# ChaoyueSong/MoDA

Measured on AMD Instinct MI355X. Metric: rays/s (256 samples/ray, 8x256 MLP, 25 bones), higher is better.
Workload: dtype f16

## Files before the change

### moda_amd/csrc/mlp_fused.hip

```cpp
#include <hip/hip_runtime.h>
#include <stdint.h>

#include <atomic>
#include <type_traits>

#include "moda_hip.h"
#include "moda_dev.h"

namespace {

typedef float f32x16 __attribute__((ext_vector_type(16)));
typedef float f32x4 __attribute__((ext_vector_type(4)));
typedef __bf16 bf16x8 __attribute__((ext_vector_type(8)));
typedef _Float16 f16x8 __attribute__((ext_vector_type(8)));

#ifndef MODA_BF16_WAVES
#define MODA_BF16_WAVES 8
#endif
#ifndef MODA_BF16_CB128
#define MODA_BF16_CB128 2
#endif
#ifndef MODA_BF16_CB
#define MODA_BF16_CB 1
#endif
#ifndef MODA_BF16_CB64
#define MODA_BF16_CB64 1
#endif
#ifndef MODA_BF16_WAVES64
#define MODA_BF16_WAVES64 16
#endif
#ifndef MODA_RING
#define MODA_RING 6
#endif
#ifndef MODA_STAGGER
#define MODA_STAGGER 0
#endif
#ifndef MODA_RESIDENT
#define MODA_RESIDENT 1
#endif
#ifndef MODA_APIPE
#define MODA_APIPE 2
#endif
#ifndef MODA_HEAD_PREFETCH
#define MODA_HEAD_PREFETCH 0
#endif
#ifndef MODA_DMA_LEADERS
#define MODA_DMA_LEADERS 0
#endif
#ifndef MODA_DMA_SPLIT
#define MODA_DMA_SPLIT 0
#endif
#ifndef MODA_XLAYER
#define MODA_XLAYER 0
#endif
#ifndef MODA_X3_EPI_PIPE
#define MODA_X3_EPI_PIPE 0
#endif
#ifndef MODA_X3_WAVES256
#define MODA_X3_WAVES256 4
#endif
#ifndef MODA_X3_WAVES128
#define MODA_X3_WAVES128 4
#endif
#ifndef MODA_X3_WAVES
#define MODA_X3_WAVES 8
#endif
#ifndef MODA_RING_SAFE
#define MODA_RING_SAFE 1
#endif
#ifndef MODA_F16_TRACK
#define MODA_F16_TRACK 1
#endif
#ifndef MODA_AGPR_APIPE
#define MODA_AGPR_APIPE 4
#endif
#ifndef MODA_AGPR_PREFETCH
#define MODA_AGPR_PREFETCH 0
// ... 704 lines not shown
        return (qi & 2) ? -r : r;
    }
    static DEVINL void encode(Pe& p, float x, float y, float z, int h, const float* win_lds) {
        float v[32];
#pragma unroll
        for (int q = 0; q < 30; ++q) {
            const int k = q / 3;
            const int c = q - 3 * k;
            const float t = (c == 0 ? x : (c == 1 ? y : z)) * (float)(1 << k);
            v[q] = win_lds[k] * sin_quarter_shifted(t, h);
        }
        v[30] = h ? y : x;
        v[31] = h ? 0.f : z;
#pragma unroll
        for (int g = 0; g < PEG; ++g) {
            union { u32x4_ w; bf16x8 b; } oh, ol;
#pragma unroll
            for (int q = 0; q < 4; ++q) {
                unsigned hi, lo;
                split_pk(v[8 * g + 2 * q], v[8 * g + 2 * q + 1], hi, lo);
                oh.w[q] = hi;
                ol.w[q] = lo;
            }
            p.hi[g] = oh.b;
            p.lo[g] = ol.b;
        }
    }
};

DEVINL float sigmoidf(float v) { return 1.f / (1.f + expf(-v)); }
DEVINL void keep_alive(const f32x16& v) { asm volatile("" ::"v"(v)); }

template <int W, typename P, int CB, int NWAVES, bool ENDY, bool UNI, bool WARP = false, int DUMP = 0, int RING = MODA_RING,
          bool COMP = false, bool HX = false>
__global__ __launch_bounds__(NWAVES * 64) __attribute__((amdgpu_waves_per_eu(NWAVES / 4, NWAVES / 4)))
void mlp_fused_kernel(MlpArgs a) {
    static_assert(!HX || (kIsF16<P> && ((WARP && W == 64) || (!WARP && W == 256 && DUMP == 0 && !COMP))),
                  "split heads: the fp16 skin + warp kernel and the fp16 8 x 256 kernel");
    constexpr bool HXR = HX && !WARP;
    static_assert(!COMP || (UNI && !WARP && DUMP == 0 && CB == 1 && std::is_same<P, PrecBF16>::value),
                  "the compositing epilogue is built for the bf16 UNI inference kernels");
    static_assert(!WARP || (UNI && !std::is_same<P, PrecF32>::value), "the warp epilogue is built for the bf16-geometry UNI kernels");
    static_assert(!DUMP || (std::is_same<P, PrecBF16>::value && !WARP), "activation dumps are built for the bf16 kernels");
    constexpr int NTHREADS = NWAVES * 64;
    constexpr int NT = W / 32;
    constexpr int NTD = (NT / 2 > 0) ? NT / 2 : 1;
    constexpr int CHF = (W == 64) ? 8 : 16;
    constexpr int TILE = NWAVES * 32 * CB;
    constexpr bool RESIDENT = (W == 64) && kIs16<P> && (MODA_RESIDENT != 0);
    using RingT = Ring<CHF, NWAVES, RESIDENT, RING, kAsmMfma<P>>;
    const int ring_chunks = RESIDENT ? a.nchunks : RING;

    extern __shared__ __attribute__((aligned(16))) unsigned char smem[];
    float* bias_lds = (float*)(smem + ring_chunks * RingT::kChunkBytes);
    float* win_lds = bias_lds + a.nbias;
    constexpr int RBW = 2 * W + NTD * 32;
    float* rb_slots = win_lds + 16;
    f32x4* pe_lds = (f32x4*)(rb_slots + NWAVES * CB * RBW) + threadIdx.x;
    constexpr int PE_VEC = sizeof(typename P::Pe) / 16;
    constexpr int TBW = (DUMP == 4) ? 2048 : 4096;
    constexpr int TBRS = (DUMP == 4) ? 64 : 128;
    unsigned char* const tbuf = (unsigned char*)(rb_slots + NWAVES * CB * RBW) + sizeof(typename P::Pe) * CB * NTHREADS +
                                (threadIdx.x >> 6) * (CB * TBW);

    const int lane = threadIdx.x & 63;
    const int wave = __builtin_amdgcn_readfirstlane(threadIdx.x >> 6);
    const int col = lane & 31;
    const int h = lane >> 5;

    for (int i = threadIdx.x; i < a.nbias; i += NTHREADS) bias_lds[i] = a.bias[i];
    if (threadIdx.x < 16) win_lds[threadIdx.x] = a.window[threadIdx.x];
    __syncthreads();

    RingT ring;
    ring.rsrc = __builtin_amdgcn_make_buffer_rsrc((void*)a.wstream, 0, a.nchunks * RingT::kChunkBytes, 0x00020000);
    ring.lds = smem;
    ring.nchunks = a.nchunks;
    ring.lane = lane;
    ring.wave = wave;
    ring.leader = wave < NWAVES / 2;
    ring.prime();
    constexpr int PREQ = (kAsmMfma<P> && MODA_AGPR_PREQ != 0) ? MODA_AGPR_APIPE : 0;
    typename P::Frag preq[PREQ > 0 ? PREQ : 1];
    auto prefetch_next = [&]() __attribute__((always_inline)) {
        if constexpr (PREQ > 0) {
#pragma unroll
            for (int d = 0; d < PREQ; ++d) preq[d] = P::fetch(ring);
        }
    };
    prefetch_next();

    const bool with_sigma = (a.flags & (MODA_MLP_WITH_SIGMA | MODA_MLP_SIGMA_ONLY)) != 0;
    const bool sigma_only = (a.flags & MODA_MLP_SIGMA_ONLY) != 0;
    const bool do_sigmoid = (a.flags & MODA_MLP_SIGMOID) != 0;
    const int nout_t = (a.n_out + 31) >> 5;
    const int n_mid = a.n_pre + 1 + a.n_post;

#ifdef MODA_STAMPS
    unsigned long long stamp_acc[16] = {0};
    unsigned long long stamp_prev;
    asm volatile("s_memtime %0\n\ts_waitcnt lgkmcnt(0)" : "=s"(stamp_prev)::"memory");
#endif
    const int ntiles = (a.M + TILE - 1) / TILE;
    unsigned trk = 0u;
    struct Head {
        float x, y, z;
        f32x4 rb[3];
    };
    auto sample_at = [&](int t, int cb, bool& ok) __attribute__((always_inline)) {
        const int mm = t * TILE + wave * (32 * CB) + cb * 32 + col;
        ok = mm < a.M;
        return ok ? mm : a.M - 1;
    };
    auto row_at = [&](int t, int cb, int div, int R) __attribute__((always_inline)) {
        bool ok;
        const unsigned r = (unsigned)sample_at(t, cb, ok) / (unsigned)div;
        return (int)(r < (unsigned)R ? r : (unsigned)R - 1u);
    };
    auto load_head = [&](int t, int cb, bool uni) __attribute__((always_inline)) {
        Head hd;
        hd.rb[0] = hd.rb[1] = hd.rb[2] = f32x4{0.f, 0.f, 0.f, 0.f};
        int r1u = __builtin_amdgcn_readfirstlane(row_at(t, cb, a.div1, a.R1));
        const int rdu = __builtin_amdgcn_readfirstlane(row_at(t, cb, a.divd, a.Rd));
        if constexpr (WARP) {
            if (a.rows_at_runs) r1u = a.run_start[r1u];
        }
#ifndef MODA_ABL_NOHEADLOAD
        if (uni) {
            if (lane < W / 4) {
                hd.rb[0] = *(const f32x4*)(a.rb1 + (long long)r1u * W + 4 * lane);
                hd.rb[1] = *(const f32x4*)(a.rb5 + (long long)r1u * W + 4 * lane);
            }
            if (lane < NTD * 8 && (a.flags & MODA_MLP_SIGMA_ONLY) == 0)
                hd.rb[2] = *(const f32x4*)(a.rbd + (long long)rdu * (NTD * 32) + 4 * lane);
        }
#endif
        bool ok;
        const long long mm = sample_at(t, cb, ok);
#ifdef MODA_ABL_NOHEADLOAD
        hd.x = 0.001f * (float)(mm & 1023);
        hd.y = 0.002f * (float)(lane);
        hd.z = 0.3f;
#else
        hd.x = a.xyz[mm * 3 + 0];
        hd.y = a.xyz[mm * 3 + 1];
        hd.z = a.xyz[mm * 3 + 2];
#endif
        if (a.flip != nullptr && a.flip[mm]) hd.x = -hd.x;
        return hd;
    };
    constexpr bool PREFETCH = UNI && ((MODA_HEAD_PREFETCH != 0) || (kAsmMfma<P> && MODA_AGPR_PREFETCH != 0)) && (DUMP == 0);
    Head head[CB];
    if (PREFETCH) {
#pragma unroll
        for (int cb = 0; cb < CB; ++cb) head[cb] = load_head(blockIdx.x, cb, true);
    }
    for (int tile = blockIdx.x; tile < ntiles; tile += gridDim.x) {
        STAMP(15);
        if (UNI && a.n_live != nullptr) {
            bool any_live = false;
#pragma unroll
            for (int cb = 0; cb < CB; ++cb) {
                const int m_first = tile * TILE + wave * (32 * CB) + cb * 32;
                if (m_first < a.M) {
                    const int ray = m_first / a.live_S;
                    any_live = any_live || (m_first - ray * a.live_S) < a.n_live[ray];
                }
            }
            if (!__builtin_amdgcn_readfirstlane((int)any_live)) {
                for (int c = 0; c < a.nchunks; ++c) {
                    ring.acquire();
                    ring.issue_rest();
                    ring.advance();
                }
                if (PREFETCH) {
#pragma unroll
                    for (int cb = 0; cb < CB; ++cb) head[cb] = load_head(tile + gridDim.x, cb, true);
                }
                continue;
            }
        }
        auto sample_of = [&](int cb, bool& ok) __attribute__((always_inline)) { return sample_at(tile, cb, ok); };
        auto row_of = [&](int cb, int div, int R) __attribute__((always_inline)) { return row_at(tile, cb, div, R); };
        bool rb_uni[CB];
#pragma unroll
        for (int cb = 0; cb < CB; ++cb) {
            if (UNI) {
                rb_uni[cb] = true;
            } else {
                const int r1 = row_of(cb, a.div1, a.R1), rd = row_of(cb, a.divd, a.Rd);
                const int r1u = __builtin_amdgcn_readfirstlane(r1), rdu = __builtin_amdgcn_readfirstlane(rd);
                rb_uni[cb] = __builtin_amdgcn_ballot_w64(r1 != r1u || rd != rdu) == 0ull;
            }
            if (!PREFETCH) head[cb] = load_head(tile, cb, rb_uni[cb]);
        }
        typename P::Pe pe[CB];
#pragma unroll
        for (int cb = 0; cb < CB; ++cb) P::encode(pe[cb], head[cb].x, head[cb].y, head[cb].z, h, win_lds);
#pragma unroll
        for (int cb = 0; cb < CB; ++cb) {
            float* slot = rb_slots + (wave * CB + cb) * RBW;
            if (rb_uni[cb]) {
                if (lane < W / 4) {
                    *(f32x4*)(slot + 4 * lane) = head[cb].rb[0];
                    *(f32x4*)(slot + W + 4 * lane) = head[cb].rb[1];
                }
                if (lane < NTD * 8) *(f32x4*)(slot + 2 * W + 4 * lane) = head[cb].rb[2];
            }
        }
        if (PREFETCH) {
#pragma unroll
            for (int cb = 0; cb < CB; ++cb) head[cb] = load_head(tile + gridDim.x, cb, true);
        }
        float comp_z = 0.f, comp_delta = 0.f, comp_noise_v = 0.f, comp_ib = 0.f;
        if constexpr (COMP) {
            bool okc;
            const int mmc = sample_of(0, okc);
            const int nc = mmc / a.comp_S, sxc = mmc - nc * a.comp_S;
            comp_z = a.comp_zv[mmc];
            comp_delta = (sxc + 1 < a.comp_S ? a.comp_zv[mmc + 1] - comp_z : 1e10f) * comp_dnorm(a.comp_rd, nc);
            comp_noise_v = a.comp_noise ? a.comp_noise[mmc] : 0.f;
            comp_ib = comp_ibeta(a.comp_beta);
        }
        STAMP(0);

        typename P::Act actX[CB][NT], actY[CB][NT];
#pragma unroll
        for (int cb = 0; cb < CB; ++cb)
#pragma unroll
            for (int t = 0; t < NT; ++t) {
                P::fresh_act(actX[cb][t]);
                P::fresh_act(actY[cb][t]);
                if constexpr (kAsmMfma<P>) {
                    actX[cb][t].base = P::kRegX + cb * P::kRegBlock + t * P::kRegTile;
                    actY[cb][t].base = P::kRegY + cb * P::kRegBlock + t * P::kRegTile;
                }
            }

        auto init_glob = [&](f32x16& c, const float* rb, int row, int ld, int rt) __attribute__((always_inline)) {
            const float* p = rb + (long long)row * ld + 32 * rt + 4 * h;
#pragma unroll
            for (int q = 0; q < 4; ++q) {
                const f32x4 v = *(const f32x4*)(p + 8 * q);
#pragma unroll
                for (int i = 0; i < 4; ++i) c[4 * q + i] = v[i];
// ... 297 lines not shown
            if constexpr (PREQ > 0) {
                ring.end_layer();
                prefetch_next();
            }
#pragma unroll
            for (int cb = 0; cb < CB; ++cb) settle_acc<P>(accs[cb]);
        }
        if constexpr (PREQ == 0) ring.end_layer();
#pragma unroll
        for (int cb = 0; cb < CB; ++cb) P::note(trk, accs[cb][0]);
        if (sigma_only) {
#pragma unroll
            for (int cb = 0; cb < CB; ++cb) {
                bool ok;
                const long long mm = sample_of(cb, ok);
                if (ok && h == 0) a.out[mm * a.out_stride] = accs[cb][0];
            }
            continue;
        }
        boff += (NT + 1) * 32;
        STAMP(7);

        typename P::Act actd[CB][NTD];
        if constexpr (kAsmMfma<P>) {
            static_assert(!kAsmMfma<P> || (CB == 2 && NT == 8 && NWAVES == 4 && !WARP && DUMP == 0 && !COMP), "the AGPR map of PrecBF16A / PrecF16A");
#pragma unroll
            for (int cb = 0; cb < CB; ++cb)
#pragma unroll
                for (int t = 0; t < NTD; ++t) {
                    actd[cb][t].base = (ENDY ? P::kRegX : P::kRegY) + cb * P::kRegBlock + t * P::kRegTile;
                    if constexpr (HXR) actd_lo[cb][t].base = actd[cb][t].base + NTD * P::kRegTile;
                }
        }
        f32x16 acco[CB][2];
        if constexpr (HX && WARP) {
            f32x16 accd[CB];
#pragma unroll
            for (int cb = 0; cb < CB; ++cb) init_rowbias(accd[cb], cb, 2, 0);
#pragma unroll
            for (int t = 0; t < NT; ++t)
#pragma unroll
                for (int sb = 0; sb < P::SUBS; ++sb) {
                    const f32x4 whi = ring.next(), wlo = ring.next();
#pragma unroll
                    for (int cb = 0; cb < CB; ++cb) {
                        accd[cb] = __builtin_amdgcn_mfma_f32_32x32x16_f16(P::as_f16(wlo), hid[cb][t].b[sb], accd[cb], 0, 0, 0);
                        accd[cb] = __builtin_amdgcn_mfma_f32_32x32x16_f16(P::as_f16(whi), hid[cb][t].b[sb], accd[cb], 0, 0, 0);
                    }
                }
            ring.end_layer();
            typename P::Act actd_lo[CB];
#pragma unroll
            for (int cb = 0; cb < CB; ++cb) {
                P::note(trk, accd[cb][0]);
#pragma unroll
                for (int u = 0; u < 2; ++u) {
                    union { typename P::u32x4 w; f16x8 b; } oh, ol;
#pragma unroll
                    for (int q = 0; q < 4; ++q) {
                        const float v0 = fmaxf(accd[cb][8 * u + 2 * q], 0.f), v1 = fmaxf(accd[cb][8 * u + 2 * q + 1], 0.f);
                        const unsigned hi = P::cvt_pk(v0, v1);
                        union { unsigned u; _Float16 h[2]; } hh;
                        hh.u = hi;
                        oh.w[q] = hi;
                        ol.w[q] = P::cvt_pk(v0 - (float)hh.h[0], v1 - (float)hh.h[1]);
                    }
                    actd[cb][0].b[u] = oh.b;
                    actd_lo[cb].b[u] = ol.b;
                }
            }
#pragma unroll
            for (int ot = 0; ot < 2; ++ot)
#pragma unroll
                for (int cb = 0; cb < CB; ++cb) init_lds(acco[cb][ot], bias_lds + boff, ot);
#pragma unroll
            for (int ot = 0; ot < 2; ++ot) {
                if (ot < nout_t) {
#pragma unroll
                    for (int sb = 0; sb < P::SUBS; ++sb) {
                        const f32x4 whi = ring.next(), wlo = ring.next();
#pragma unroll
                        for (int cb = 0; cb < CB; ++cb) {
                            acco[cb][ot] = __builtin_amdgcn_mfma_f32_32x32x16_f16(P::as_f16(wlo), actd[cb][0].b[sb], acco[cb][ot], 0, 0, 0);
                            acco[cb][ot] = __builtin_amdgcn_mfma_f32_32x32x16_f16(P::as_f16(whi), actd_lo[cb].b[sb], acco[cb][ot], 0, 0, 0);
                            acco[cb][ot] = __builtin_amdgcn_mfma_f32_32x32x16_f16(P::as_f16(whi), actd[cb][0].b[sb], acco[cb][ot], 0, 0, 0);
                        }
                    }
                }
            }
            ring.end_layer();
        } else {
        layer(hid, actd, IC_NTD{}, IC_NT{}, false, true, 2, 0, true, DUMP ? a.dump_dd : nullptr, NTD * 32, false, false, HXR);
        STAMP(8);
#pragma unroll
        for (int ot = 0; ot < 2; ++ot)
#pragma unroll
            for (int cb = 0; cb < CB; ++cb) init_lds(acco[cb][ot], bias_lds + boff, ot);
#pragma unroll
        for (int ot = 0; ot < 2; ++ot) {
            if (ot < nout_t) {
#pragma unroll
                for (int cb = 0; cb < CB; ++cb) guard_acc<P>(acco[cb][ot]);
#pragma unroll
                for (int t = 0; t < NTD; ++t)
#pragma unroll
                    for (int sb = 0; sb < P::SUBS; ++sb) {
                        if constexpr (HXR) {
                            const f32x4 whi = ring.next(), wlo = ring.next();
#pragma unroll
                            for (int cb = 0; cb < CB; ++cb) {
// ... 54 lines not shown
            CompTerms q;
            const float w = comp_sample_terms(alpha, T, live, sx + 1 >= S, cr, cg, cbv, z, 0.f, 0.f, 0.f,
                                              (live && a.comp_cyc) ? a.comp_cyc[mm] : 0.f, &q);
            if (live) {
                if (a.comp_out.weights) a.comp_out.weights[mm] = w;
                if (a.comp_out.visibility) a.comp_out.visibility[mm] = T;
            }
            const float gr = comp_group_sum(q.r), gg = comp_group_sum(q.g), gb = comp_group_sum(q.b), gd = comp_group_sum(q.d),
                        gs = comp_group_sum(q.s), gc = comp_group_sum(q.c);
            if (lane == 0) {
                float* rec = cx + wave * 8;
                rec[1] = gr; rec[2] = gg; rec[3] = gb; rec[4] = gd; rec[5] = gs; rec[6] = gc;
            }
            asm volatile("s_waitcnt lgkmcnt(0)\n\ts_barrier" ::: "memory");
            if (g == 0 && lane == 0 && ok) {
#pragma clang fp contract(off)
                float ar = 0.f, ag = 0.f, ab = 0.f, ad = 0.f, as = 0.f, ac = 0.f;
                for (int k = 0; k < gpr; ++k) {
                    const float* rec = cx + (wave + k) * 8;
                    ar = ar + rec[1]; ag = ag + rec[2]; ab = ab + rec[3]; ad = ad + rec[4]; as = as + rec[5]; ac = ac + rec[6];
                }
                a.comp_out.rgb[n * 3 + 0] = ar; a.comp_out.rgb[n * 3 + 1] = ag; a.comp_out.rgb[n * 3 + 2] = ab;
                a.comp_out.depth[n] = ad;
                a.comp_out.sil[n] = as;
                if (a.comp_out.cyc_out && a.comp_cyc) a.comp_out.cyc_out[n] = ac;
            }
            continue;
        }
        if constexpr (WARP) {
#pragma unroll
            for (int cb = 0; cb < CB; ++cb) {
                bool ok;
                const int mm = sample_of(cb, ok);
                const int m_first = __builtin_amdgcn_readfirstlane(tile * TILE + wave * (32 * CB) + cb * 32);
                const int ray = min(m_first, a.M - 1) / a.warp_S;
                long long qset = a.q_rps > 0 ? ray / a.q_rps : 0;
                long long dset = ray / a.dq_rps;
                if (a.run_start != nullptr) {
                    dset = a.run_start[dset];
                    if (a.q_rps > 0) qset = a.run_start[qset];
                }
                const float* qt = a.qtab + qset * nout_t * kWarpQFloats + lane;
                const f32x4* dt = a.dqtab + dset * nout_t * (kWarpDqFrags * 64) + lane;
                float qa[2][kWarpQFrags];
                f32x4 da[2][kWarpDqFrags];
#pragma unroll
                for (int ot = 0; ot < 2; ++ot) {
                    const int o2 = ot < nout_t ? ot : 0;
#pragma unroll
                    for (int f = 0; f < kWarpQFrags; ++f) qa[ot][f] = qt[(o2 * kWarpQFrags + f) * 64];
#pragma unroll
                    for (int u = 0; u < kWarpDqFrags; ++u) da[ot][u] = dt[(o2 * kWarpDqFrags + u) * 64];
                }
                const float x = a.xyz[(long long)mm * 3 + 0], y = a.xyz[(long long)mm * 3 + 1], z = a.xyz[(long long)mm * 3 + 2];
                float mono[kWarpQFrags] = {h ? y * y : x * x, h ? x * y : z * z, h ? y * z : x * z, h ? y : x, h ? 1.f : z};
#pragma unroll
                for (int ot = 0; ot < 2; ++ot)
                    if (ot < nout_t) {
#pragma unroll
                        for (int f = 0; f < kWarpQFrags; ++f)
                            acco[cb][ot] = __builtin_amdgcn_mfma_f32_32x32x2f32(qa[ot][f], mono[f], acco[cb][ot], 0, 0, 0);
                    }
                float mx = -INFINITY;
#pragma unroll
                for (int ot = 0; ot < 2; ++ot)
                    if (ot < nout_t) {
#pragma unroll
                        for (int i = 0; i < 16; ++i) mx = fmaxf(mx, acco[cb][ot][i]);
                    }
#pragma unroll
                for (int f = 0; f < kWarpQFrags; ++f) asm volatile("" ::"v"(mono[f]), "v"(qa[0][f]), "v"(qa[1][f]), "v"(mx));
                {
                    unsigned ma = __builtin_bit_cast(unsigned, mx), mb = ma;
                    asm volatile("" : "+v"(mb));
                    const auto mr = __builtin_amdgcn_permlane32_swap(ma, mb, false, false);
                    const unsigned m0 = mr[0], m1 = mr[1];
                    mx = fmaxf(__uint_as_float(m0), __uint_as_float(m1));
                }
                const float kLog2e = 1.4426950408889634f;
                const float nmx = -mx * kLog2e;
                typedef unsigned u32x4 __attribute__((ext_vector_type(4)));
                union Pack { u32x4 w; bf16x8 b; };
                Pack whi[2][2], wlo[2][2];
                auto pack_tile = [&](int ot) __attribute__((always_inline)) {
#pragma unroll
                    for (int u = 0; u < 2; ++u)
#pragma unroll
                        for (int q = 0; q < 4; ++q) {
                            const float e0 = __builtin_amdgcn_exp2f(__builtin_fmaf(acco[cb][ot][8 * u + 2 * q], kLog2e, nmx));
                            const float e1 = __builtin_amdgcn_exp2f(__builtin_fmaf(acco[cb][ot][8 * u + 2 * q + 1], kLog2e, nmx));
                            const unsigned ph = PrecBF16::cvt_pk(e0, e1);
                            whi[ot][u].w[q] = ph;
                            wlo[ot][u].w[q] = PrecBF16::cvt_pk(e0 - __builtin_bit_cast(float, ph << 16),
                                                               e1 - __builtin_bit_cast(float, ph & 0xffff0000u));
                        }
                };
                pack_tile(0);
                if (nout_t > 1) {
                    pack_tile(1);
                } else {
#pragma unroll
                    for (int u = 0; u < 2; ++u) whi[1][u].w = wlo[1][u].w = u32x4{0u, 0u, 0u, 0u};
                }
                f32x16 bl;
#pragma unroll
                for (int i = 0; i < 16; ++i) bl[i] = 0.f;
                __builtin_amdgcn_sched_barrier(0);
#pragma unroll
                for (int ot = 0; ot < 2; ++ot)
                    if (ot < nout_t) {
#pragma unroll
                        for (int u = 0; u < 2; ++u) {
                            bl = __builtin_amdgcn_mfma_f32_32x32x16_bf16(PrecBF16::as_bf16(da[ot][u]), whi[ot][u].b, bl, 0, 0, 0);
                            bl = __builtin_amdgcn_mfma_f32_32x32x16_bf16(PrecBF16::as_bf16(da[ot][u]), wlo[ot][u].b, bl, 0, 0, 0);
                        }
                    }
                __builtin_amdgcn_sched_barrier(0);
                float c8[8];
#pragma unroll
                for (int k = 0; k < 4; ++k) {
                    const float lo4 = bl[k] + bl[4 + k], hi4 = bl[8 + k] + bl[12 + k];
                    c8[k] = h ? hi4 : lo4;
                    c8[4 + k] = h ? lo4 : hi4;
                }
#pragma unroll
                for (int ot = 0; ot < 2; ++ot)
#pragma unroll
                    for (int u = 0; u < 2; ++u)
                        asm volatile("" ::"v"(whi[ot][u].w), "v"(wlo[ot][u].w), "v"(da[ot][u]), "v"(c8[0]), "v"(c8[1]), "v"(c8[2]),
                                     "v"(c8[3]), "v"(c8[4]), "v"(c8[5]), "v"(c8[6]), "v"(c8[7]));
                float px = x, py = y, pz = z;
                if (a.pts_tf != nullptr) {
                    px = a.pts_tf[(long long)mm * 3 + 0]; py = a.pts_tf[(long long)mm * 3 + 1]; pz = a.pts_tf[(long long)mm * 3 + 2];
                }
                float ox, oy, oz;
#ifdef MODA_WARP_EXACT_DIV
                dqs_apply(c8, px, py, pz, &ox, &oy, &oz);
#else
                dqs_apply_fast(c8, px, py, pz, &ox, &oy, &oz);
#endif
                if (ok && h == 0) {
                    if (a.out != nullptr) {
                        float* o = a.out + (long long)mm * 3;
                        o[0] = ox; o[1] = oy; o[2] = oz;
                    }
                    if (a.cyc_ref != nullptr) {
                        const float dx = a.cyc_ref[(long long)mm * 3 + 0] - ox, dy = a.cyc_ref[(long long)mm * 3 + 1] - oy,
                                    dz = a.cyc_ref[(long long)mm * 3 + 2] - oz;
                        a.cyc_out[mm] = __builtin_amdgcn_sqrtf(dx * dx + dy * dy + dz * dz);
                    }
                }
            }
            continue;
        }
#ifdef MODA_ABL_NOSTORE
#pragma unroll
        for (int cb = 0; cb < CB; ++cb) { keep_alive(acco[cb][0]); keep_alive(acco[cb][1]); keep_alive(accs[cb]); }
        continue;
#endif
#pragma unroll
        for (int cb = 0; cb < CB; ++cb) {
            bool ok;
            const int mm = sample_of(cb, ok);
            if (!ok) continue;
            if (a.n_out == 3 && with_sigma && a.out_tr_S == 0 && a.out_stride == 4) {
                if (h == 0) {
                    f32x4 v;
#pragma unroll
                    for (int i = 0; i < 3; ++i) v[i] = do_sigmoid ? sigmoidf(acco[cb][0][i]) : acco[cb][0][i];
                    v[3] = accs[cb][0];
                    *(f32x4*)(a.out + (long long)mm * 4) = v;
                }
                continue;
            }
            float* o = a.out + (long long)mm * a.out_stride;
            int rs = 1;
            if (a.out_tr_S > 0) {
                const int ray = (unsigned)mm / (unsigned)a.out_tr_S;
                o = a.out + (long long)ray * a.out_stride * a.out_tr_S + (mm - ray * a.out_tr_S);
                rs = a.out_tr_S;
                const int m_first = tile * TILE + wave * (32 * CB) + cb * 32;
#ifndef MODA_ABL_NO_TRSTORE
                if ((a.out_tr_S & 31) == 0 && m_first + 31 < a.M && !with_sigma) {
                    float* tb = (float*)(pe_lds - threadIdx.x) + (long long)cb * PE_VEC * NTHREADS * 4 + wave * 256;
// ... 71 lines not shown
    const bool f16 = (d->flags & MODA_MLP_F16) != 0;
    if ((int)x3 + (int)f16 + (int)((d->flags & MODA_MLP_BF16) != 0) > 1) return MODA_EINVAL;
    const bool bf16 = x3 || f16 || (d->flags & MODA_MLP_BF16) != 0;
    const bool sigma_only = (d->flags & MODA_MLP_SIGMA_ONLY) != 0;
    const bool with_sigma = sigma_only || (d->flags & MODA_MLP_WITH_SIGMA) != 0;
    s->chf = d->W == 64 ? 8 : 16;
    s->subs = bf16 ? 2 : 4;
    s->peg = bf16 ? 4 : 8;
    s->nt = d->W / 32;
    s->ntd = s->nt / 2 > 0 ? s->nt / 2 : 1;
    const long long m = x3 ? 2 : 1;
    const bool hx = (d->flags & MODA_MLP_F16_HEADS) != 0;
    if (hx && (!f16 || sigma_only || (d->W == 64 && with_sigma) || d->W == 128)) return MODA_EINVAL;
    const long long mh = hx ? 2 : m;
    const long long mdir = (hx && d->W == 256) ? m : mh;
    const long long act = m * s->nt * s->nt * s->subs;
    const long long pef = m * s->peg * s->nt;
    long long c = 0;
    c += pad_to(pef, s->chf);
    c += 3 * pad_to(act, s->chf);
    c += pad_to(pef + act, s->chf);
    c += (long long)(d->D - 5) * pad_to(act, s->chf);
    c += pad_to(with_sigma ? m * s->nt * s->subs : 0, s->chf);
    if (!sigma_only) {
        c += pad_to(mdir * s->ntd * s->nt * s->subs, s->chf);
        c += pad_to(mh * ((d->n_out + 31) / 32) * s->ntd * s->subs, s->chf);
    }
    s->chunks = c / s->chf;
    s->nbias = (long long)(d->D - 2) * d->W + (s->nt + 1) * 32 + 64;
    return 0;
}

template <int W, typename P, int CB, int NWAVES, bool ENDY, bool UNI, bool WARP = false, int DUMP = 0, int RING = MODA_RING,
          bool COMP = false, bool HX = false>
static int launch_p(const MlpArgs& a, hipStream_t stream) {
    constexpr int CHF = (W == 64) ? 8 : 16;
    constexpr int TILE = NWAVES * 32 * CB;
    const size_t pe_bytes = sizeof(typename P::Pe) * CB * NWAVES * 64;
    constexpr bool RESIDENT = (W == 64) && kIs16<P> && (MODA_RESIDENT != 0);
    const size_t ring_chunks = RESIDENT ? (size_t)a.nchunks : (size_t)RING;
    constexpr int NTD = (W / 64 > 0) ? W / 64 : 1;
    const size_t rb_bytes = (size_t)NWAVES * CB * (2 * W + NTD * 32) * sizeof(float);
    const size_t lds = ring_chunks * CHF * kFragBytes + (size_t)(a.nbias + 16) * sizeof(float) + rb_bytes + pe_bytes +
                       (DUMP == 3 ? (size_t)NWAVES * CB * 4096 : (DUMP == 4 ? (size_t)NWAVES * CB * 2048 : 0));
    if (lds > 160 * 1024) return MODA_ESHAPE;
    static std::atomic<unsigned long long> attr_set{0ull};
    int devid = 0;
    if (hipGetDevice(&devid) != hipSuccess) devid = 0;
    const unsigned long long bit = 1ull << (devid & 63);
    if (devid > 63 || !(attr_set.load(std::memory_order_relaxed) & bit)) {
        hipError_t e = hipFuncSetAttribute((const void*)mlp_fused_kernel<W, P, CB, NWAVES, ENDY, UNI, WARP, DUMP, RING, COMP, HX>,
                                           hipFuncAttributeMaxDynamicSharedMemorySize, 160 * 1024);
        if (e != hipSuccess) return (int)e;
        attr_set.fetch_or(bit, std::memory_order_relaxed);
    }
    const long long ntiles = ((long long)a.M + TILE - 1) / TILE;
    int grid = ntiles < 256 ? (int)ntiles : 256;
    if (grid < 1) return 0;
    hipLaunchKernelGGL((mlp_fused_kernel<W, P, CB, NWAVES, ENDY, UNI, WARP, DUMP, RING, COMP, HX>), dim3(grid), dim3(NWAVES * 64), lds, stream, a);
    return (int)hipGetLastError();
}

template <int W, typename P, int CB, int NWAVES, int DUMP = 0, int RING = MODA_RING, bool HX = false>
static int launch(const MlpArgs& a, hipStream_t stream) {
    const bool uni = (a.R1 == 1 || a.div1 % 32 == 0) && (a.Rd == 1 || a.divd % 32 == 0);
    const bool endy = ((a.n_pre + 1 + a.n_post) & 1) != 0;
    if (uni)
        return endy ? launch_p<W, P, CB, NWAVES, true, true, false, DUMP, RING, false, HX>(a, stream)
                    : launch_p<W, P, CB, NWAVES, false, true, false, DUMP, RING, false, HX>(a, stream);
    return endy ? launch_p<W, P, CB, NWAVES, true, false, false, DUMP, RING, false, HX>(a, stream)
                : launch_p<W, P, CB, NWAVES, false, false, false, DUMP, RING, false, HX>(a, stream);
}

}

#ifdef MODA_STAMPS
extern "C" int moda_dbg_read_stamps(unsigned long long* host16) {
    if (!moda_dbg_stamps_ptr) return -1;
    hipDeviceSynchronize();
    return (int)hipMemcpy(host16, moda_dbg_stamps_ptr, 16 * sizeof(unsigned long long), hipMemcpyDeviceToHost);
}
#endif

extern "C" int64_t moda_mlp_stream_bytes(const moda_mlp_desc* d) {
    StreamShape s;
    if (stream_shape(d, &s) != 0) return -1;
    return s.chunks * s.chf * kFragBytes;
}

extern "C" int64_t moda_mlp_bias_floats(const moda_mlp_desc* d) {
    StreamShape s;
    if (stream_shape(d, &s) != 0) return -1;
    return s.nbias;
}

template <typename P>
static int wide128(const MlpArgs& a, hipStream_t st) {
    const bool uni = (a.R1 == 1 || a.div1 % 32 == 0) && (a.Rd == 1 || a.divd % 32 == 0);
    const bool endy = ((a.n_pre + 1 + a.n_post) & 1) != 0;
    if (MODA_BF16_CB128 > 1 && uni && !endy && a.M >= 256 * 512 && a.n_live == nullptr)
        return launch_p<128, P, (MODA_BF16_CB128 > 1 ? MODA_BF16_CB128 : 1), MODA_BF16_WAVES, false, true, false, 0, 4>(a, st);
    return launch<128, P, MODA_BF16_CB, MODA_BF16_WAVES>(a, st);
}

// ... 168 lines not shown

extern "C" int moda_mlp_warp_fwd(const moda_mlp_desc* d, const void* wstream, const float* bias, const float* xyz,
                                 const float* rb1, const float* rb5, int64_t R1, int64_t div1, const float* rbd, const float* qtab,
                                 int64_t q_rps, const void* dqtab, int64_t dq_rps, const float* pts_tf, const float* cyc_ref, float* xyz_out,
                                 float* cyc_out, int64_t S, int64_t M, const int32_t* run_start, void* stream) {
    if (!d) return MODA_EINVAL;
    if (d->W != 64 || !(d->flags & (MODA_MLP_BF16 | MODA_MLP_F16 | MODA_MLP_BF16X3)) ||
        (d->flags & (MODA_MLP_SIGMA_ONLY | MODA_MLP_WITH_SIGMA | MODA_MLP_SIGMOID)))
        return MODA_ESHAPE;
    if (S < 32 || S % 32 != 0 || M % S != 0 || q_rps < 0 || dq_rps < 1) return MODA_ESHAPE;
    if (M <= 0) return 0;
    if (!qtab || !dqtab || (!xyz_out && !cyc_ref) || (cyc_ref && !cyc_out) || !rb1 || !rb5 || !rbd) return MODA_EINVAL;
    if (R1 != 1 && div1 % 32 != 0) return MODA_ESHAPE;
    MlpArgs a;
    float dummy_out = 0.f;
    const int rc = fill_args(d, wstream, bias, xyz, nullptr, rb1, rb5, R1, div1, rbd, 1, 1, xyz_out ? xyz_out : &dummy_out, 3, 0, M, stream, &a);
    if (rc != 0) return rc;
    a.out = xyz_out;
    a.qtab = qtab;
    a.dqtab = (const f32x4*)dqtab;
    a.pts_tf = pts_tf;
    a.cyc_ref = cyc_ref;
    a.cyc_out = cyc_out;
    a.warp_S = (int)S;
    a.q_rps = (int)(q_rps > 0x7fffffff ? 0x7fffffff : q_rps);
    a.dq_rps = (int)(dq_rps > 0x7fffffff ? 0x7fffffff : dq_rps);
    if (run_start && q_rps > 0 && q_rps != dq_rps) return MODA_EINVAL;
    if (d->reserved & MODA_MLP_ROWS_AT_RUNS) {
        if (!run_start || R1 <= 1 || div1 != S * dq_rps) return MODA_EINVAL;
        a.rows_at_runs = 1;
    }
    a.run_start = (const int*)run_start;
    constexpr int NW = MODA_RESIDENT ? MODA_BF16_WAVES64 : MODA_BF16_WAVES;
    const bool endy = ((a.n_pre + 1 + a.n_post) & 1) != 0;
    hipStream_t st = (hipStream_t)stream;
    if (d->flags & MODA_MLP_F16_HEADS)
        return endy ? launch_p<64, PrecF16, MODA_BF16_CB64, NW, true, true, true, 0, MODA_RING, false, true>(a, st)
                    : launch_p<64, PrecF16, MODA_BF16_CB64, NW, false, true, true, 0, MODA_RING, false, true>(a, st);
    if (d->flags & MODA_MLP_F16)
        return endy ? launch_p<64, PrecF16, MODA_BF16_CB64, NW, true, true, true>(a, st)
                    : launch_p<64, PrecF16, MODA_BF16_CB64, NW, false, true, true>(a, st);
    if (d->flags & MODA_MLP_BF16X3)
        return endy ? launch_p<64, PrecBF16x3, 1, MODA_X3_WAVES, true, true, true>(a, st)
                    : launch_p<64, PrecBF16x3, 1, MODA_X3_WAVES, false, true, true>(a, st);
    return endy ? launch_p<64, PrecBF16, MODA_BF16_CB64, NW, true, true, true>(a, st)
                : launch_p<64, PrecBF16, MODA_BF16_CB64, NW, false, true, true>(a, st);
}

extern "C" int moda_mlp_dump_fwd(const moda_mlp_desc* d, const void* wstream, const float* bias, const float* xyz,
                                 const uint8_t* flip_x, const float* rb1, const float* rb5, int64_t R1, int64_t div1,
                                 const float* rbd, int64_t Rd, int64_t divd, float* out, int64_t out_stride, float* dump_h,
                                 float* dump_dd, int64_t M, void* stream) {
    if (!d) return MODA_EINVAL;
    if (!(d->flags & MODA_MLP_BF16) || (d->flags & MODA_MLP_SIGMA_ONLY)) return MODA_ESHAPE;
    if (d->W != 64 && d->W != 128 && d->W != 256) return MODA_ESHAPE;
    if (M <= 0) {
        StreamShape s;
        return stream_shape(d, &s);
    }
    if (!dump_h || !dump_dd) return MODA_EINVAL;
    if ((long long)M * d->W * 4 >= (1LL << 32)) return MODA_ESHAPE;
    MlpArgs a;
    const int rc = fill_args(d, wstream, bias, xyz, flip_x, rb1, rb5, R1, div1, rbd, Rd, divd, out, out_stride, 0, M, stream, &a);
    if (rc != 0) return rc;
    a.dump_h = dump_h;
    a.dump_dd = dump_dd;
    a.dump_bf16 = (d->reserved & MODA_MLP_DUMP_BF16) != 0;
    hipStream_t st = (hipStream_t)stream;
#ifndef MODA_DUMP_MODE
#define MODA_DUMP_MODE 3
#endif
    if (a.dump_bf16) {
#ifndef MODA_DUMP_MODE256
#define MODA_DUMP_MODE256 2
#endif
#if MODA_DUMP_MODE256 == 4
        if (d->W == 256) return launch<256, PrecBF16, MODA_BF16_CB, MODA_BF16_WAVES, 4, MODA_RING - 1>(a, st);
#endif
        if (d->W == 256) return launch<256, PrecBF16, MODA_BF16_CB, MODA_BF16_WAVES, 2>(a, st);
// ... 12 lines not shown
```

Measured before the change: 4.098 million.

## Cache warp bone tables across tiles with contiguous tile ranges and compile-time bone-tile count

Result: no change. 4.132 million (median of 6 runs) (+0.8%).

```diff
diff --git a/moda_amd/csrc/mlp_fused.hip b/moda_amd/csrc/mlp_fused.hip
--- a/moda_amd/csrc/mlp_fused.hip
+++ b/moda_amd/csrc/mlp_fused.hip
@@ -43,6 +43,9 @@
 #endif
 #ifndef MODA_HEAD_PREFETCH
 #define MODA_HEAD_PREFETCH 0
+#endif
+#ifndef MODA_WARP_KEEP
+#define MODA_WARP_KEEP 1
 #endif
 #ifndef MODA_DMA_LEADERS
 #define MODA_DMA_LEADERS 0
@@ -813,9 +816,10 @@
 DEVINL void keep_alive(const f32x16& v) { asm volatile("" ::"v"(v)); }
 
 template <int W, typename P, int CB, int NWAVES, bool ENDY, bool UNI, bool WARP = false, int DUMP = 0, int RING = MODA_RING,
-          bool COMP = false, bool HX = false>
+          bool COMP = false, bool HX = false, int BT = 2>
 __global__ __launch_bounds__(NWAVES * 64) __attribute__((amdgpu_waves_per_eu(NWAVES / 4, NWAVES / 4)))
 void mlp_fused_kernel(MlpArgs a) {
+    static_assert(BT == 2 || (WARP && BT == 1), "one or two bone tiles; the one-tile form exists for the warp kernels only");
     static_assert(!HX || (kIsF16<P> && ((WARP && W == 64) || (!WARP && W == 256 && DUMP == 0 && !COMP))),
                   "split heads: the fp16 skin + warp kernel and the fp16 8 x 256 kernel");
     constexpr bool HXR = HX && !WARP;
@@ -874,7 +878,7 @@
     const bool with_sigma = (a.flags & (MODA_MLP_WITH_SIGMA | MODA_MLP_SIGMA_ONLY)) != 0;
     const bool sigma_only = (a.flags & MODA_MLP_SIGMA_ONLY) != 0;
     const bool do_sigmoid = (a.flags & MODA_MLP_SIGMOID) != 0;
-    const int nout_t = (a.n_out + 31) >> 5;
+    const int nout_t = WARP ? BT : (a.n_out + 31) >> 5;
     const int n_mid = a.n_pre + 1 + a.n_post;
 
 #ifdef MODA_STAMPS
@@ -932,11 +936,36 @@
     };
     constexpr bool PREFETCH = UNI && ((MODA_HEAD_PREFETCH != 0) || (kAsmMfma<P> && MODA_AGPR_PREFETCH != 0)) && (DUMP == 0);
     Head head[CB];
+    int tile0 = blockIdx.x, tile_end = ntiles;
+    const unsigned tstep = WARP ? 1u : gridDim.x;
+    if constexpr (WARP) {
+        const int per = ntiles / (int)gridDim.x, rem = ntiles - per * (int)gridDim.x;
+        tile0 = (int)blockIdx.x * per + min((int)blockIdx.x, rem);
+        tile_end = tile0 + per + ((int)blockIdx.x < rem ? 1 : 0);
+    }
+    constexpr int WBT = WARP ? BT : 1, WCB = WARP ? CB : 1;
+    float wq[WCB][WBT][kWarpQFrags];
+    f32x4 wd[WCB][WBT][kWarpDqFrags];
+    int w_qset[WCB], w_dset[WCB];
+#pragma unroll
+    for (int cb = 0; cb < WCB; ++cb) w_qset[cb] = w_dset[cb] = -1;
+    auto warp_sets = [&](int t, int cb, int& qset, int& dset) __attribute__((always_inline)) {
+        const int m_first = __builtin_amdgcn_readfirstlane(t * TILE + wave * (32 * CB) + cb * 32);
+        const int ray = min(m_first, a.M - 1) / a.warp_S;
+        qset = a.q_rps > 0 ? ray / a.q_rps : 0;
+        dset = ray / a.dq_rps;
+        if (a.run_start != nullptr) {
+            dset = a.run_start[dset];
+            if (a.q_rps > 0) qset = a.run_start[qset];
+        }
+        qset = __builtin_amdgcn_readfirstlane(qset);
+        dset = __builtin_amdgcn_readfirstlane(dset);
+    };
     if (PREFETCH) {
 #pragma unroll
-        for (int cb = 0; cb < CB; ++cb) head[cb] = load_head(blockIdx.x, cb, true);
-    }
-    for (int tile = blockIdx.x; tile < ntiles; tile += gridDim.x) {
+        for (int cb = 0; cb < CB; ++cb) head[cb] = load_head(tile0, cb, true);
+    }
+    for (int tile = tile0; tile < tile_end; tile += tstep) {
         STAMP(15);
         if (UNI && a.n_live != nullptr) {
             bool any_live = false;
@@ -956,7 +985,7 @@
                 }
                 if (PREFETCH) {
 #pragma unroll
-                    for (int cb = 0; cb < CB; ++cb) head[cb] = load_head(tile + gridDim.x, cb, true);
+                    for (int cb = 0; cb < CB; ++cb) head[cb] = load_head(tile + tstep, cb, true);
                 }
                 continue;
             }
@@ -975,6 +1004,31 @@
             }
             if (!PREFETCH) head[cb] = load_head(tile, cb, rb_uni[cb]);
         }
+        float wx[WCB], wy[WCB], wz[WCB];
+        if constexpr (WARP) {
+#pragma unroll
+            for (int cb = 0; cb < CB; ++cb) {
+                int qs, ds;
+                warp_sets(tile, cb, qs, ds);
+                if (!MODA_WARP_KEEP || qs != w_qset[cb]) {
+                    const float* qt = a.qtab + (long long)qs * BT * kWarpQFloats + lane;
+#pragma unroll
+                    for (int ot = 0; ot < BT; ++ot)
+#pragma unroll
+                        for (int f = 0; f < kWarpQFrags; ++f) wq[cb][ot][f] = qt[(ot * kWarpQFrags + f) * 64];
+                    w_qset[cb] = qs;
+                }
+                if (!MODA_WARP_KEEP || ds != w_dset[cb]) {
+                    const f32x4* dt = a.dqtab + (long long)ds * BT * (kWarpDqFrags * 64) + lane;
+#pragma unroll
+                    for (int ot = 0; ot < BT; ++ot)
+#pragma unroll
+                        for (int u = 0; u < kWarpDqFrags; ++u) wd[cb][ot][u] = dt[(ot * kWarpDqFrags + u) * 64];
+                    w_dset[cb] = ds;
+                }
+                wx[cb] = head[cb].x; wy[cb] = head[cb].y; wz[cb] = head[cb].z;
+            }
+        }
         typename P::Pe pe[CB];
 #pragma unroll
         for (int cb = 0; cb < CB; ++cb) P::encode(pe[cb], head[cb].x, head[cb].y, head[cb].z, h, win_lds);
@@ -991,7 +1045,7 @@
         }
         if (PREFETCH) {
 #pragma unroll
-            for (int cb = 0; cb < CB; ++cb) head[cb] = load_head(tile + gridDim.x, cb, true);
+            for (int cb = 0; cb < CB; ++cb) head[cb] = load_head(tile + tstep, cb, true);
         }
         float comp_z = 0.f, comp_delta = 0.f, comp_noise_v = 0.f, comp_ib = 0.f;
         if constexpr (COMP) {
@@ -1355,6 +1409,18 @@
                     if constexpr (HXR) actd_lo[cb][t].base = actd[cb][t].base + NTD * P::kRegTile;
                 }
         }
+        float wpx[WCB], wpy[WCB], wpz[WCB];
+        if constexpr (WARP) {
+#pragma unroll
+            for (int cb = 0; cb < CB; ++cb) {
+                wpx[cb] = wx[cb]; wpy[cb] = wy[cb]; wpz[cb] = wz[cb];
+                if (a.pts_tf != nullptr) {
+                    bool ok;
+                    const long long mm = sample_of(cb, ok);
+                    wpx[cb] = a.pts_tf[mm * 3 + 0]; wpy[cb] = a.pts_tf[mm * 3 + 1]; wpz[cb] = a.pts_tf[mm * 3 + 2];
+                }
+            }
+        }
         f32x16 acco[CB][2];
         if constexpr (HX && WARP) {
             f32x16 accd[CB];
@@ -1393,12 +1459,12 @@
                 }
             }
 #pragma unroll
-            for (int ot = 0; ot < 2; ++ot)
+            for (int ot = 0; ot < BT; ++ot)
 #pragma unroll
                 for (int cb = 0; cb < CB; ++cb) init_lds(acco[cb][ot], bias_lds + boff, ot);
 #pragma unroll
-            for (int ot = 0; ot < 2; ++ot) {
-                if (ot < nout_t) {
+            for (int ot = 0; ot < BT; ++ot) {
+                {
 #pragma unroll
                     for (int sb = 0; sb < P::SUBS; ++sb) {
                         const f32x4 whi = ring.next(), wlo = ring.next();
@@ -1519,44 +1585,34 @@
             for (int cb = 0; cb < CB; ++cb) {
                 bool ok;
                 const int mm = sample_of(cb, ok);
-                const int m_first = __builtin_amdgcn_readfirstlane(tile * TILE + wave * (32 * CB) + cb * 32);
-                const int ray = min(m_first, a.M - 1) / a.warp_S;
-                long long qset = a.q_rps > 0 ? ray / a.q_rps : 0;
-                long long dset = ray / a.dq_rps;
-                if (a.run_start != nullptr) {
-                    dset = a.run_start[dset];
-                    if (a.q_rps > 0) qset = a.run_start[qset];
-                }
-                const float* qt = a.qtab + qset * nout_t * kWarpQFloats + lane;
-                const f32x4* dt = a.dqtab + dset * nout_t * (kWarpDqFrags * 64) + lane;
-                float qa[2][kWarpQFrags];
-                f32x4 da[2][kWarpDqFrags];
-#pragma unroll
-                for (int ot = 0; ot < 2; ++ot) {
-                    const int o2 = ot < nout_t ? ot : 0;
-#pragma unroll
-                    for (int f = 0; f < kWarpQFrags; ++f) qa[ot][f] = qt[(o2 * kWarpQFrags + f) * 64];
-#pragma unroll
-                    for (int u = 0; u < kWarpDqFrags; ++u) da[ot][u] = dt[(o2 * kWarpDqFrags + u) * 64];
-                }
-                const float x = a.xyz[(long long)mm * 3 + 0], y = a.xyz[(long long)mm * 3 + 1], z = a.xyz[(long long)mm * 3 + 2];
+                auto& qa = wq[cb];
+                auto& da = wd[cb];
+                const float x = wx[cb], y = wy[cb], z = wz[cb];
                 float mono[kWarpQFrags] = {h ? y * y : x * x, h ? x * y : z * z, h ? y * z : x * z, h ? y : x, h ? 1.f : z};
-#pragma unroll
-                for (int ot = 0; ot < 2; ++ot)
-                    if (ot < nout_t) {
-#pragma unroll
-                        for (int f = 0; f < kWarpQFrags; ++f)
-                            acco[cb][ot] = __builtin_amdgcn_mfma_f32_32x32x2f32(qa[ot][f], mono[f], acco[cb][ot], 0, 0, 0);
-                    }
+#ifdef MODA_STAMPS
+#pragma unroll
+                for (int ot = 0; ot < BT; ++ot) {
+#pragma unroll
+                    for (int f = 0; f < kWarpQFrags; ++f) asm volatile("" ::"v"(qa[ot][f]), "v"(mono[f]));
+#pragma unroll
+                    for (int u = 0; u < kWarpDqFrags; ++u) asm volatile("" ::"v"(da[ot][u]));
+                }
+#endif
+                STAMP(11);
+#pragma unroll
+                for (int ot = 0; ot < BT; ++ot) {
+#pragma unroll
+                    for (int f = 0; f < kWarpQFrags; ++f)
+                        acco[cb][ot] = __builtin_amdgcn_mfma_f32_32x32x2f32(qa[ot][f], mono[f], acco[cb][ot], 0, 0, 0);
+                }
                 float mx = -INFINITY;
 #pragma unroll
-                for (int ot = 0; ot < 2; ++ot)
-                    if (ot < nout_t) {
-#pragma unroll
-                        for (int i = 0; i < 16; ++i) mx = fmaxf(mx, acco[cb][ot][i]);
-                    }
-#pragma unroll
-                for (int f = 0; f < kWarpQFrags; ++f) asm volatile("" ::"v"(mono[f]), "v"(qa[0][f]), "v"(qa[1][f]), "v"(mx));
+                for (int ot = 0; ot < BT; ++ot) {
+#pragma unroll
+                    for (int i = 0; i < 16; ++i) mx = fmaxf(mx, acco[cb][ot][i]);
+                }
+#pragma unroll
+                for (int f = 0; f < kWarpQFrags; ++f) asm volatile("" ::"v"(mono[f]), "v"(qa[0][f]), "v"(qa[BT - 1][f]), "v"(mx));
                 {
                     unsigned ma = __builtin_bit_cast(unsigned, mx), mb = ma;
                     asm volatile("" : "+v"(mb));
@@ -1568,7 +1624,7 @@
                 const float nmx = -mx * kLog2e;
                 typedef unsigned u32x4 __attribute__((ext_vector_type(4)));
                 union Pack { u32x4 w; bf16x8 b; };
-                Pack whi[2][2], wlo[2][2];
+                Pack whi[BT][2], wlo[BT][2];
                 auto pack_tile = [&](int ot) __attribute__((always_inline)) {
 #pragma unroll
                     for (int u = 0; u < 2; ++u)
@@ -1582,26 +1638,21 @@
                                                                e1 - __builtin_bit_cast(float, ph & 0xffff0000u));
                         }
                 };
-                pack_tile(0);
-                if (nout_t > 1) {
-                    pack_tile(1);
-                } else {
-#pragma unroll
-                    for (int u = 0; u < 2; ++u) whi[1][u].w = wlo[1][u].w = u32x4{0u, 0u, 0u, 0u};
-                }
+#pragma unroll
+                for (int ot = 0; ot < BT; ++ot) pack_tile(ot);
+                STAMP(12);
                 f32x16 bl;
 #pragma unroll
                 for (int i = 0; i < 16; ++i) bl[i] = 0.f;
                 __builtin_amdgcn_sched_barrier(0);
 #pragma unroll
-                for (int ot = 0; ot < 2; ++ot)
-                    if (ot < nout_t) {
-#pragma unroll
-                        for (int u = 0; u < 2; ++u) {
-                            bl = __builtin_amdgcn_mfma_f32_32x32x16_bf16(PrecBF16::as_bf16(da[ot][u]), whi[ot][u].b, bl, 0, 0, 0);
-                            bl = __builtin_amdgcn_mfma_f32_32x32x16_bf16(PrecBF16::as_bf16(da[ot][u]), wlo[ot][u].b, bl, 0, 0, 0);
-                        }
+                for (int ot = 0; ot < BT; ++ot) {
+#pragma unroll
+                    for (int u = 0; u < 2; ++u) {
+                        bl = __builtin_amdgcn_mfma_f32_32x32x16_bf16(PrecBF16::as_bf16(da[ot][u]), whi[ot][u].b, bl, 0, 0, 0);
+                        bl = __builtin_amdgcn_mfma_f32_32x32x16_bf16(PrecBF16::as_bf16(da[ot][u]), wlo[ot][u].b, bl, 0, 0, 0);
                     }
+                }
                 __builtin_amdgcn_sched_barrier(0);
                 float c8[8];
 #pragma unroll
@@ -1611,21 +1662,22 @@
                     c8[4 + k] = h ? lo4 : hi4;
                 }
 #pragma unroll
-                for (int ot = 0; ot < 2; ++ot)
+                for (int ot = 0; ot < BT; ++ot)
 #pragma unroll
                     for (int u = 0; u < 2; ++u)
                         asm volatile("" ::"v"(whi[ot][u].w), "v"(wlo[ot][u].w), "v"(da[ot][u]), "v"(c8[0]), "v"(c8[1]), "v"(c8[2]),
                                      "v"(c8[3]), "v"(c8[4]), "v"(c8[5]), "v"(c8[6]), "v"(c8[7]));
-                float px = x, py = y, pz = z;
-                if (a.pts_tf != nullptr) {
-                    px = a.pts_tf[(long long)mm * 3 + 0]; py = a.pts_tf[(long long)mm * 3 + 1]; pz = a.pts_tf[(long long)mm * 3 + 2];
-                }
+                const float px = wpx[cb], py = wpy[cb], pz = wpz[cb];
                 float ox, oy, oz;
 #ifdef MODA_WARP_EXACT_DIV
                 dqs_apply(c8, px, py, pz, &ox, &oy, &oz);
 #else
                 dqs_apply_fast(c8, px, py, pz, &ox, &oy, &oz);
 #endif
+#ifdef MODA_STAMPS
+                asm volatile("" ::"v"(ox), "v"(oy), "v"(oz));
+#endif
+                STAMP(13);
                 if (ok && h == 0) {
                     if (a.out != nullptr) {
                         float* o = a.out + (long long)mm * 3;
@@ -1637,6 +1689,7 @@
                         a.cyc_out[mm] = __builtin_amdgcn_sqrtf(dx * dx + dy * dy + dz * dz);
                     }
                 }
+                STAMP(14);
             }
             continue;
         }
@@ -1774,7 +1827,7 @@
 }
 
 template <int W, typename P, int CB, int NWAVES, bool ENDY, bool UNI, bool WARP = false, int DUMP = 0, int RING = MODA_RING,
-          bool COMP = false, bool HX = false>
+          bool COMP = false, bool HX = false, int BT = 2>
 static int launch_p(const MlpArgs& a, hipStream_t stream) {
     constexpr int CHF = (W == 64) ? 8 : 16;
     constexpr int TILE = NWAVES * 32 * CB;
@@ -1791,7 +1844,7 @@
     if (hipGetDevice(&devid) != hipSuccess) devid = 0;
     const unsigned long long bit = 1ull << (devid & 63);
     if (devid > 63 || !(attr_set.load(std::memory_order_relaxed) & bit)) {
-        hipError_t e = hipFuncSetAttribute((const void*)mlp_fused_kernel<W, P, CB, NWAVES, ENDY, UNI, WARP, DUMP, RING, COMP, HX>,
+        hipError_t e = hipFuncSetAttribute((const void*)mlp_fused_kernel<W, P, CB, NWAVES, ENDY, UNI, WARP, DUMP, RING, COMP, HX, BT>,
                                            hipFuncAttributeMaxDynamicSharedMemorySize, 160 * 1024);
         if (e != hipSuccess) return (int)e;
         attr_set.fetch_or(bit, std::memory_order_relaxed);
@@ -1799,7 +1852,7 @@
     const long long ntiles = ((long long)a.M + TILE - 1) / TILE;
     int grid = ntiles < 256 ? (int)ntiles : 256;
     if (grid < 1) return 0;
-    hipLaunchKernelGGL((mlp_fused_kernel<W, P, CB, NWAVES, ENDY, UNI, WARP, DUMP, RING, COMP, HX>), dim3(grid), dim3(NWAVES * 64), lds, stream, a);
+    hipLaunchKernelGGL((mlp_fused_kernel<W, P, CB, NWAVES, ENDY, UNI, WARP, DUMP, RING, COMP, HX, BT>), dim3(grid), dim3(NWAVES * 64), lds, stream, a);
     return (int)hipGetLastError();
 }
 
@@ -1812,6 +1865,16 @@
                     : launch_p<W, P, CB, NWAVES, false, true, false, DUMP, RING, false, HX>(a, stream);
     return endy ? launch_p<W, P, CB, NWAVES, true, false, false, DUMP, RING, false, HX>(a, stream)
                 : launch_p<W, P, CB, NWAVES, false, false, false, DUMP, RING, false, HX>(a, stream);
+}
+
+template <typename P, int CB, int NWAVES, bool HX>
+static int launch_warp(const MlpArgs& a, hipStream_t stream) {
+    const bool endy = ((a.n_pre + 1 + a.n_post) & 1) != 0;
+    if ((a.n_out + 31) / 32 == 1)
+        return endy ? launch_p<64, P, CB, NWAVES, true, true, true, 0, MODA_RING, false, HX, 1>(a, stream)
+                    : launch_p<64, P, CB, NWAVES, false, true, true, 0, MODA_RING, false, HX, 1>(a, stream);
+    return endy ? launch_p<64, P, CB, NWAVES, true, true, true, 0, MODA_RING, false, HX, 2>(a, stream)
+                : launch_p<64, P, CB, NWAVES, false, true, true, 0, MODA_RING, false, HX, 2>(a, stream);
 }
 
 }
@@ -2046,19 +2109,11 @@
     }
     a.run_start = (const int*)run_start;
     constexpr int NW = MODA_RESIDENT ? MODA_BF16_WAVES64 : MODA_BF16_WAVES;
-    const bool endy = ((a.n_pre + 1 + a.n_post) & 1) != 0;
     hipStream_t st = (hipStream_t)stream;
-    if (d->flags & MODA_MLP_F16_HEADS)
-        return endy ? launch_p<64, PrecF16, MODA_BF16_CB64, NW, true, true, true, 0, MODA_RING, false, true>(a, st)
-                    : launch_p<64, PrecF16, MODA_BF16_CB64, NW, false, true, true, 0, MODA_RING, false, true>(a, st);
-    if (d->flags & MODA_MLP_F16)
-        return endy ? launch_p<64, PrecF16, MODA_BF16_CB64, NW, true, true, true>(a, st)
-                    : launch_p<64, PrecF16, MODA_BF16_CB64, NW, false, true, true>(a, st);
-    if (d->flags & MODA_MLP_BF16X3)
-        return endy ? launch_p<64, PrecBF16x3, 1, MODA_X3_WAVES, true, true, true>(a, st)
-                    : launch_p<64, PrecBF16x3, 1, MODA_X3_WAVES, false, true, true>(a, st);
-    return endy ? launch_p<64, PrecBF16, MODA_BF16_CB64, NW, true, true, true>(a, st)
-                : launch_p<64, PrecBF16, MODA_BF16_CB64, NW, false, true, true>(a, st);
+    if (d->flags & MODA_MLP_F16_HEADS) return launch_warp<PrecF16, MODA_BF16_CB64, NW, true>(a, st);
+    if (d->flags & MODA_MLP_F16) return launch_warp<PrecF16, MODA_BF16_CB64, NW, false>(a, st);
+    if (d->flags & MODA_MLP_BF16X3) return launch_warp<PrecBF16x3, 1, MODA_X3_WAVES, false>(a, st);
+    return launch_warp<PrecBF16, MODA_BF16_CB64, NW, false>(a, st);
 }
 
 extern "C" int moda_mlp_dump_fwd(const moda_mlp_desc* d, const void* wstream, const float* bias, const float* xyz,
```
